# PX4/disparity_to_point_cloud

Measured on NVIDIA B200. Metric: Mpixels/s disparity->PointCloud2, higher is better.
Workload: dtype f64

## Files before the change

disparity_to_point_cloud_b200/csrc/capi.cu:

```cuda
#include "../../include/d2pc_b200.h"

#include <algorithm>
#include <atomic>
#include <cfloat>
#include <cmath>
#include <cstdio>
#include <cstdlib>
#include <cstring>
#include <mutex>
#include <new>
#include <string>
#include <utility>
#include <vector>

#include <nvtx3/nvToolsExt.h>
#include <sys/mman.h>

#include "cloud_transform.h"
#include "crop_box.h"
#include "fusion.h"
#include "laser_scan.h"
#include "median.h"
#include "radius_outlier.h"
#include "reproject.h"
// ... 49 lines not shown
  DevBuf d_in, d_out;
  StageBufs stages;
  DevBuf d_fuse_in[4], d_pre[2], d_container, d_combined, d_fused;
  DevBuf d_ranges;
  PinBuf h_ranges;
  uint32_t *d_count = nullptr;
  uint32_t *h_count = nullptr;
  cudaEvent_t ev_h2d = nullptr, ev_kernel = nullptr, ev_d2h = nullptr;
  cudaEvent_t ev_start = nullptr;
  bool timed = false;
  cudaStream_t s_kern = nullptr;
  bool pending = false;
  CloudPlan plan;
  uint8_t *user_dst = nullptr;
  size_t user_cap = 0;
  bool user_pinned = false;
  bool late_copy = false;
};

}

struct d2pc_ctx {
  d2pc_config cfg;
  int device = 0;
  int sm_count = 148;
  cudaStream_t s_h2d = nullptr, s_compute = nullptr, s_d2h = nullptr;
  double q[16];
  QParams Q;
  std::vector<Slot> slots;
  uint32_t epoch = 0;
  uint64_t launches = 0;
  std::string last_cuda_error;
  StageBufs batch;
  uint32_t *d_ticket = nullptr;
  d2pc_voxel_grid voxel;
  bool voxel_set = false;
  d2pc_radius_outlier ror;
  d2pc_crop_box box;
  d2pc_cloud_transform xform;
  d2pc_laser_scan_params scan;
  ScanPlan scan_plan;
  d2pc_laser_scan last_scan{};
  bool last_scan_on = false;
  DevBuf d_fuse_in[4], d_container, d_combined, d_fused;
  PinBuf h_fused, h_combined;
  DevBuf d_score_in, d_score_out[2];
  PinBuf h_score[2];
  DevBuf d_color_in, d_color_out, d_color_lut;
  PinBuf h_color;
  PinBuf h_stage;
  bool color_lut_ready = false;
  cudaEvent_t ev_fuse = nullptr;
  int rows_per_unit = 0, ctas_per_sm = 0, median_strip = 0, median_variant = 0;
  bool force_scalar = false, force_generic = false;
  int compact_variant = 0, exact_variant = 0, prefetch_dist = 0, zero_numer = 0, crop_load = 0, crop_probe = 0;
  int fuse_median = 0;
  int direct_out = 0;
  bool timing = false;
  std::vector<std::pair<uintptr_t, bool>> pin_cache;
  uint64_t pin_cache_gen = 0;
};

namespace {

struct NvtxRange {
  explicit NvtxRange(const char *name) { nvtxRangePushA(name); }
  ~NvtxRange() { nvtxRangePop(); }
};

std::atomic<uint64_t> g_host_gen{1};

int cuda_fail(d2pc_ctx *ctx, cudaError_t e, const char *what) {
  if (ctx) {
    ctx->last_cuda_error = std::string(what) + ": " + cudaGetErrorString(e);
  }
  if (e == cudaErrorMemoryAllocation) return D2PC_ERR_NOMEM;
  if (e == cudaErrorNoDevice || e == cudaErrorInsufficientDriver || e == cudaErrorInvalidDevice)
    return D2PC_ERR_NO_DEVICE;
  return D2PC_ERR_CUDA;
}

#define CU(ctx, call)                                      \
  do {                                                     \
    cudaError_t e__ = (call);                              \
    if (e__ != cudaSuccess) return cuda_fail(ctx, e__, #call); \
  } while (0)

int grow_dev(d2pc_ctx *ctx, DevBuf &b, size_t bytes, cudaStream_t clear_on = nullptr) {
  if (bytes <= b.cap) return D2PC_OK;
  if (b.p) CU(ctx, cudaFree(b.p));
  b.p = nullptr;
  b.cap = 0;
  const size_t cap = round_up(bytes, 1 << 16);
  CU(ctx, cudaMalloc(&b.p, cap));
  if (clear_on) CU(ctx, cudaMemsetAsync(b.p, 0, cap, clear_on));
  b.cap = cap;
  return D2PC_OK;
}
struct HostBlock {
  void *p;
  size_t bytes;
};
std::mutex g_thp_mutex;
std::vector<HostBlock> g_thp_blocks;

cudaError_t pinned_alloc(void **out, size_t bytes) {
// ... 287 lines not shown
}

int enqueue_reproject(d2pc_ctx *ctx, const CloudPlan &p, const FrameBatch &in, StageBufs &b, const CloudDst &dst,
                      uint32_t *ticket, cudaStream_t stream) {
  const d2pc_config &c = ctx->cfg;
  int nl = 0;
  ReprojectLaunch L;
  L.in = in.data;
  L.in_is_f32 = in.is_f32;
  L.step = in.step;
  L.frame_stride = in.frame_stride;
  L.n_frames = in.n_frames;
  L.width = in.w;
  L.height = in.h;
  L.border = c.border;
  L.scale = c.disparity_scale;
  L.out = dst.points;
  L.out_stride_bytes = dst.stride;
  L.counts = dst.counts;
  L.Q = &ctx->Q;
  L.arith_fast = c.arith_mode == D2PC_ARITH_FAST;
  L.compact = p.compact;
  L.scratch = b.scratch.p;
  L.tables = b.tables.p;
  L.ticket = ticket;
  L.sm_count = ctx->sm_count;
  L.rows_per_unit = ctx->rows_per_unit;
  L.ctas_per_sm = ctx->ctas_per_sm;
  L.force_scalar = ctx->force_scalar;
  L.force_generic = ctx->force_generic;
  L.compact_variant = ctx->compact_variant;
  L.exact_variant = ctx->exact_variant;
  L.zero_numer = ctx->zero_numer;
  L.prefetch_dist = ctx->prefetch_dist;
  L.crop_load = ctx->crop_load;
  L.crop_probe = ctx->crop_probe != 0;
  if (!in.is_f32 && c.median_ksize > 1) {
    MedianLaunch M;
    M.src = in.data;
    M.dst = b.med.p;
    M.src_step = M.dst_step = in.step;
    M.src_frame_stride = M.dst_frame_stride = in.frame_stride;
    M.n_frames = in.n_frames;
    M.width = (int)in.w;
    M.height = (int)in.h;
    M.ox0 = c.border;
    M.oy0 = c.border;
    M.ow = (int)in.w - 2 * c.border;
    M.oh = (int)in.h - 2 * c.border;
    M.ksize = c.median_ksize;
    M.sm_count = ctx->sm_count;
    M.strip_rows = ctx->median_strip;
    M.variant = ctx->median_variant;
    bool zero_numer = false;
    const bool fuse = ctx->fuse_median >= 0 && M.ow > 0 && M.oh > 0 && (c.median_ksize > 3 || M.variant != 0) &&
                      reproject_fuses_with_median(L, &zero_numer);
    if (fuse) {
      M.zero_numer = zero_numer;
      M.points = dst.points;
      M.points_stride_bytes = dst.stride;
      M.Q = &ctx->Q;
      M.scale = c.disparity_scale;
    }
    CU(ctx, launch_median_u8(M, stream, &nl));
    ctx->launches += nl;
    if (fuse) return D2PC_OK;
    L.in = b.med.p;
  }
  L.epoch = L.compact ? next_epoch(ctx) : 0;
  CU(ctx, launch_reproject(L, stream, &nl));
  ctx->launches += nl;
  return D2PC_OK;
}

int enqueue_kernels(d2pc_ctx *ctx, const CloudPlan &p, const FrameBatch &in, StageBufs &b, const CloudDst &out,
                    uint32_t *fallback, uint32_t *ticket, cudaStream_t stream, float *ranges = nullptr) {
  const uint32_t n = (uint32_t)p.n;
  const int stages = p.n_stages;
  const CloudDst buf[2] = {cloud_buf(b.cloud[0], in.n_frames, n), cloud_buf(b.cloud[1], in.n_frames, n)};
  int rc = enqueue_reproject(ctx, p, in, b, stages ? buf[0] : out, ticket, stream);
  for (int i = 0; i < stages && !rc; ++i) {
    const CloudDst &src = buf[i & 1];
    const CloudSrc cloud{src.points, src.stride, i > 0 || p.compact ? src.counts : nullptr, in.n_frames, n};
    rc = enqueue_stage(ctx, p.stages[i], cloud, i + 1 < stages ? buf[(i + 1) & 1] : out, fallback, b.stage.p, stream);
  }
  if (rc || !p.scan.on || !ranges) return rc;
  const CloudSrc cloud{out.points, out.stride, p.counted ? out.counts : nullptr, in.n_frames, n};
  int nl = 0;
  CU(ctx, launch_laser_scan(cloud, p.scan.p, ranges, (size_t)p.scan.p.n * 4, stream, &nl));
  ctx->launches += nl;
  return D2PC_OK;
}

int check_frame(const d2pc_ctx *ctx, const void *data, uint32_t w, uint32_t h, size_t step, int esz) {
  if (!ctx || !data) return D2PC_ERR_INVALID_ARG;
  if (w == 0 || h == 0 || w > (1u << 16) || h > (1u << 16)) return D2PC_ERR_BAD_DIMS;
  if (step < (size_t)w * esz) return D2PC_ERR_BAD_DIMS;
  if (esz == 4 && (step % 4 != 0 || reinterpret_cast<uintptr_t>(data) % 4 != 0)) return D2PC_ERR_BAD_DIMS;
  return D2PC_OK;
}

int slot_wait_idle(d2pc_ctx *ctx, Slot &s) {
  if (s.pending) {
    CU(ctx, cudaEventSynchronize(s.ev_d2h));
    s.pending = false;
  }
// ... 193 lines not shown
  int n = 0;
  cudaError_t e = cudaGetDeviceCount(&n);
  if (e != cudaSuccess || n == 0) {
    cudaGetLastError();
    return D2PC_ERR_NO_DEVICE;
  }
  if (device < 0 || device >= n) return D2PC_ERR_NO_DEVICE;
  int major = 0;
  cudaDeviceGetAttribute(&major, cudaDevAttrComputeCapabilityMajor, device);
  if (major != 10) return D2PC_ERR_NO_DEVICE;

  d2pc_ctx *ctx = new (std::nothrow) d2pc_ctx();
  if (!ctx) return D2PC_ERR_NOMEM;
  ctx->cfg = c;
  ctx->device = device;
  int rc = D2PC_OK;
  auto fail = [&](int code) {
    d2pc_destroy(ctx);
    return code;
  };
  if (cudaSetDevice(device) != cudaSuccess) return fail(D2PC_ERR_NO_DEVICE);
  cudaDeviceGetAttribute(&ctx->sm_count, cudaDevAttrMultiProcessorCount, device);
  if (cudaStreamCreateWithFlags(&ctx->s_h2d, cudaStreamNonBlocking) != cudaSuccess ||
      cudaStreamCreateWithFlags(&ctx->s_compute, cudaStreamNonBlocking) != cudaSuccess ||
      cudaStreamCreateWithFlags(&ctx->s_d2h, cudaStreamNonBlocking) != cudaSuccess ||
      cudaEventCreateWithFlags(&ctx->ev_fuse, cudaEventDisableTiming) != cudaSuccess)
    return fail(D2PC_ERR_CUDA);
  if (cudaMalloc(&ctx->d_ticket, 64) != cudaSuccess) return fail(D2PC_ERR_NOMEM);
  ctx->slots.resize(c.n_slots);
  for (auto &s : ctx->slots) {
    if (cudaEventCreateWithFlags(&s.ev_h2d, cudaEventDisableTiming) != cudaSuccess ||
        cudaEventCreateWithFlags(&s.ev_kernel, cudaEventDisableTiming) != cudaSuccess ||
        cudaEventCreateWithFlags(&s.ev_d2h, cudaEventDisableTiming) != cudaSuccess ||
        cudaStreamCreateWithFlags(&s.s_kern, cudaStreamNonBlocking) != cudaSuccess)
      return fail(D2PC_ERR_CUDA);
    if (cudaMalloc(&s.d_count, 64) != cudaSuccess) return fail(D2PC_ERR_NOMEM);
    if (cudaHostAlloc(&s.h_count, 64, cudaHostAllocDefault) != cudaSuccess) return fail(D2PC_ERR_NOMEM);
    cudaMemsetAsync(s.d_count, 0, 64, ctx->s_compute);
  }
  rc = d2pc_q_from_intrinsics(c.fx, c.fy, c.cx, c.cy, c.baseline, c.rect_width, c.rect_height, ctx->q);
  if (rc) return fail(rc);
  make_qparams(ctx->q, &ctx->Q);
  d2pc_voxel_grid_default(&ctx->voxel);
  d2pc_radius_outlier_default(&ctx->ror);
  d2pc_crop_box_default(&ctx->box);
  d2pc_cloud_transform_default(&ctx->xform);
  d2pc_laser_scan_params_default(&ctx->scan);
  scan_plan_of(&ctx->scan, &ctx->scan_plan);

  if (const char *v = getenv("D2PC_ROWS_PER_UNIT")) ctx->rows_per_unit = atoi(v);
  if (const char *v = getenv("D2PC_CTAS_PER_SM")) ctx->ctas_per_sm = atoi(v);
  if (const char *v = getenv("D2PC_CROP_LOAD")) ctx->crop_load = atoi(v);
  if (const char *v = getenv("D2PC_MEDIAN_STRIP")) ctx->median_strip = atoi(v);
  if (const char *v = getenv("D2PC_EXACT_VARIANT")) ctx->exact_variant = atoi(v);

  if (c.max_width > 0 && c.max_height > 0) {
    for (auto &s : ctx->slots) {
      const size_t pitch = round_up((size_t)c.max_width * 4, kAlign);
      const uint64_t np = crop_points(c.max_width, c.max_height, c.border);
      if ((rc = grow_dev(ctx, s.d_in, pitch * c.max_height)) ||
          (rc = grow_dev(ctx, s.stages.med, pitch * c.max_height)) ||
          (rc = grow_dev(ctx, s.d_out, np * 16 + 16)) || (rc = grow_pin(ctx, s.h_out, np * 16 + 16)) ||
          (rc = grow_pin(ctx, s.h_in, (size_t)c.max_width * 4 * c.max_height)))
        return fail(rc);
    }
  }
  *out = ctx;
  return D2PC_OK;
}

void d2pc_destroy(d2pc_ctx *ctx) {
  if (!ctx) return;
  cudaSetDevice(ctx->device);
  cudaDeviceSynchronize();
  for (auto &s : ctx->slots) {
    free_pin(s.h_in), free_pin(s.h_out);
    free_dev(s.d_in), free_dev(s.d_out), free_stages(s.stages), free_dev(s.d_ranges), free_pin(s.h_ranges);
    for (auto &b : s.d_fuse_in) free_dev(b);
    free_dev(s.d_pre[0]), free_dev(s.d_pre[1]), free_dev(s.d_container), free_dev(s.d_combined), free_dev(s.d_fused);
    if (s.d_count) cudaFree(s.d_count);
    if (s.h_count) cudaFreeHost(s.h_count);
    if (s.ev_h2d) cudaEventDestroy(s.ev_h2d);
    if (s.ev_kernel) cudaEventDestroy(s.ev_kernel);
    if (s.ev_d2h) cudaEventDestroy(s.ev_d2h);
    if (s.ev_start) cudaEventDestroy(s.ev_start);
    if (s.s_kern) cudaStreamDestroy(s.s_kern);
  }
  free_stages(ctx->batch);
  for (auto &b : ctx->d_fuse_in) free_dev(b);
  free_dev(ctx->d_container), free_dev(ctx->d_combined), free_dev(ctx->d_fused);
  free_pin(ctx->h_fused), free_pin(ctx->h_combined);
  free_dev(ctx->d_score_in), free_dev(ctx->d_score_out[0]), free_dev(ctx->d_score_out[1]);
  free_pin(ctx->h_score[0]), free_pin(ctx->h_score[1]);
  free_dev(ctx->d_color_in), free_dev(ctx->d_color_out), free_dev(ctx->d_color_lut), free_pin(ctx->h_color);
  free_pin(ctx->h_stage);
  if (ctx->d_ticket) cudaFree(ctx->d_ticket);
  if (ctx->ev_fuse) cudaEventDestroy(ctx->ev_fuse);
  if (ctx->s_h2d) cudaStreamDestroy(ctx->s_h2d);
  if (ctx->s_compute) cudaStreamDestroy(ctx->s_compute);
  if (ctx->s_d2h) cudaStreamDestroy(ctx->s_d2h);
  cudaGetLastError();
  delete ctx;
}

int d2pc_set_q(d2pc_ctx *ctx, const double q[16]) {
  if (!ctx || !q) return D2PC_ERR_INVALID_ARG;
// ... 88 lines not shown
  *t = ctx->xform;
  return D2PC_OK;
}
void d2pc_laser_scan_params_default(d2pc_laser_scan_params *p) {
  if (!p) return;
  memset(p, 0, sizeof(*p));
  p->struct_size = sizeof(*p);
  p->min_height = DBL_MIN, p->max_height = DBL_MAX;
  p->angle_min = -M_PI, p->angle_max = M_PI, p->angle_increment = M_PI / 180.0;
  p->scan_time = 1.0 / 30.0;
  p->range_min = 0.0, p->range_max = DBL_MAX;
  p->use_inf = 1, p->inf_epsilon = 1.0;
  p->keep_cloud = 1;
}
int d2pc_set_laser_scan(d2pc_ctx *ctx, const d2pc_laser_scan_params *p) {
  if (!ctx) return D2PC_ERR_INVALID_ARG;
  ScanPlan s;
  const int rc = scan_plan_of(p, &s);
  if (rc) return rc;
  ctx->scan = *p;
  ctx->scan_plan = s;
  return D2PC_OK;
}
int d2pc_get_laser_scan(const d2pc_ctx *ctx, d2pc_laser_scan_params *p) {
  if (!ctx || !p) return D2PC_ERR_INVALID_ARG;
  *p = ctx->scan;
  return D2PC_OK;
}
int d2pc_laser_scan_ranges(const d2pc_laser_scan_params *p, uint32_t *n) {
  ScanPlan s;
  const int rc = n ? scan_plan_of(p, &s) : D2PC_ERR_INVALID_ARG;
  if (rc) return rc;
  *n = s.msg.n_ranges;
  return D2PC_OK;
}
int d2pc_last_scan(const d2pc_ctx *ctx, d2pc_laser_scan *out) {
  if (!ctx || !out) return D2PC_ERR_INVALID_ARG;
  if (!ctx->last_scan_on) return D2PC_ERR_NOT_READY;
  *out = ctx->last_scan;
  return D2PC_OK;
}
int d2pc_set_arith_mode(d2pc_ctx *ctx, int m) {
  if (!ctx || m < 0 || m > 1) return D2PC_ERR_INVALID_ARG;
  ctx->cfg.arith_mode = m;
  return D2PC_OK;
}
int d2pc_set_tuning(d2pc_ctx *ctx, const char *key, int value) {
  if (!ctx || !key) return D2PC_ERR_INVALID_ARG;
  const std::string k(key);
  if (k == "rows_per_unit") ctx->rows_per_unit = value;
  else if (k == "ctas_per_sm") ctx->ctas_per_sm = value;
  else if (k == "median_strip") ctx->median_strip = value;
  else if (k == "median_variant") ctx->median_variant = value;
  else if (k == "force_scalar") ctx->force_scalar = value != 0;
  else if (k == "force_generic") ctx->force_generic = value != 0;
  else if (k == "force_park" || k == "compact_variant") ctx->compact_variant = value;
  else if (k == "exact_variant") ctx->exact_variant = value;
  else if (k == "zero_numer") ctx->zero_numer = value;
  else if (k == "fuse_median") ctx->fuse_median = value;
  else if (k == "direct_out") ctx->direct_out = value;
  else if (k == "prefetch_dist") ctx->prefetch_dist = value;
  else if (k == "crop_load") ctx->crop_load = value;
  else if (k == "crop_probe") ctx->crop_probe = value;
  else if (k == "median_ksize") {
    if (value < 1 || value > 15 || !(value & 1)) return D2PC_ERR_INVALID_ARG;
    ctx->cfg.median_ksize = value;
  } else if (k == "border") {
    if (value < 0) return D2PC_ERR_INVALID_ARG;
    ctx->cfg.border = value;
  } else if (k == "offset_x") ctx->cfg.offset_x = value;
  else if (k == "offset_y") ctx->cfg.offset_y = value;
  else if (k == "fuse_rule") {
    if (value < 0 || value > 7) return D2PC_ERR_INVALID_ARG;
    ctx->cfg.fuse_rule = value;
  } else if (k == "fuse_median_ksize") {
    if (value < 1 || value > 15 || !(value & 1)) return D2PC_ERR_INVALID_ARG;
    ctx->cfg.fuse_median_ksize = value;
  } else if (k == "fuse_crop_left") ctx->cfg.fuse_crop_left = value;
  else if (k == "fuse_crop_right") ctx->cfg.fuse_crop_right = value;
  else if (k == "fuse_crop_top") ctx->cfg.fuse_crop_top = value;
  else if (k == "fuse_crop_bottom") ctx->cfg.fuse_crop_bottom = value;
  else return D2PC_ERR_INVALID_ARG;
  return D2PC_OK;
}

int d2pc_submit_mono8(d2pc_ctx *ctx, int slot, const uint8_t *data, uint32_t w, uint32_t h, uint32_t step) {
  return submit_common(ctx, slot, data, w, h, step, false);
}
int d2pc_submit_f32(d2pc_ctx *ctx, int slot, const float *disp, uint32_t w, uint32_t h, uint32_t step) {
  return submit_common(ctx, slot, disp, w, h, step, true);
}

static void note_scan(d2pc_ctx *ctx, const ScanPlan &scan, const PinBuf &ranges) {
  ctx->last_scan_on = scan.on;
  ctx->last_scan = scan.msg;
  ctx->last_scan.ranges = reinterpret_cast<const float *>(ranges.p);
}

int d2pc_wait(d2pc_ctx *ctx, int slot, d2pc_cloud *out) {
  if (!ctx || slot < 0 || slot >= (int)ctx->slots.size()) return D2PC_ERR_INVALID_ARG;
  Slot &s = ctx->slots[slot];
  if (!s.pending) return D2PC_ERR_NOT_READY;
  CU(ctx, cudaSetDevice(ctx->device));
  CU(ctx, cudaEventSynchronize(s.ev_d2h));
  const uint64_t n = kept_points(s.plan, s.h_count);
  if (s.plan.counted && s.user_dst && s.user_cap < n * 16) {
// ... 254 lines not shown
  const LaserScanParams &p = ctx->scan_plan.p;
  const uint64_t bytes = (uint64_t)n_max * 16, rbytes = (uint64_t)p.n * 4;
  if (bytes > 0xffffffffull) return D2PC_ERR_BAD_DIMS;
  if (reinterpret_cast<uintptr_t>(d_in) % 16 || in_stride % 16 || reinterpret_cast<uintptr_t>(d_ranges) % 4 ||
      ranges_stride % 4 || (n_frames > 1 && (in_stride < bytes || ranges_stride < rbytes)))
    return D2PC_ERR_BAD_DIMS;
  if (n_frames == 0 || p.n == 0) return D2PC_OK;
  const uintptr_t in0 = reinterpret_cast<uintptr_t>(d_in), out0 = reinterpret_cast<uintptr_t>(d_ranges);
  const uint64_t in_end = in0 + (uint64_t)(n_frames - 1) * in_stride + bytes;
  const uint64_t out_end = out0 + (uint64_t)(n_frames - 1) * ranges_stride + rbytes;
  if (bytes && in0 < out_end && out0 < in_end) return D2PC_ERR_INVALID_ARG;
  CU(ctx, cudaSetDevice(ctx->device));
  const uint32_t chunk = frames_per_chunk(n_frames, n_max);
  for (uint32_t f0 = 0; f0 < n_frames; f0 += chunk) {
    const CloudSrc in{d_in + f0 * in_stride, in_stride, d_in_counts ? d_in_counts + f0 : nullptr,
                      std::min(chunk, n_frames - f0), n_max};
    int nl = 0;
    CU(ctx, launch_laser_scan(in, p, reinterpret_cast<float *>(reinterpret_cast<uint8_t *>(d_ranges) + f0 * ranges_stride),
                              ranges_stride, ctx->s_compute, &nl));
    ctx->launches += nl;
  }
  return D2PC_OK;
}

int d2pc_reproject_f32_device(d2pc_ctx *ctx, const float *d_disp, uint32_t n_frames, uint32_t w, uint32_t h,
                              size_t step, size_t frame_stride, uint8_t *d_points, size_t points_stride,
                              uint32_t *d_counts) {
  if (step % 4 || frame_stride % 4 || reinterpret_cast<uintptr_t>(d_disp) % 4) return D2PC_ERR_BAD_DIMS;
  return reproject_device_common(ctx, d_disp, true, n_frames, w, h, step, frame_stride, d_points, points_stride,
                                 d_counts);
}
int d2pc_reproject_mono8_device(d2pc_ctx *ctx, const uint8_t *d_img, uint32_t n_frames, uint32_t w, uint32_t h,
                                size_t step, size_t frame_stride, uint8_t *d_points, size_t points_stride,
                                uint32_t *d_counts) {
  return reproject_device_common(ctx, d_img, false, n_frames, w, h, step, frame_stride, d_points, points_stride,
                                 d_counts);
}

int d2pc_median_u8_device(d2pc_ctx *ctx, const uint8_t *d_src, uint32_t w, uint32_t h, size_t src_step,
                          uint8_t *d_dst, size_t dst_step, int ksize) {
  if (!ctx || !d_src || !d_dst) return D2PC_ERR_INVALID_ARG;
  if (w == 0 || h == 0 || src_step < w || dst_step < w) return D2PC_ERR_BAD_DIMS;
  if (ksize < 3 || ksize > 15 || !(ksize & 1)) return D2PC_ERR_INVALID_ARG;
  CU(ctx, cudaSetDevice(ctx->device));
  MedianLaunch M;
  M.src = d_src, M.dst = d_dst;
  M.src_step = src_step, M.dst_step = dst_step;
  M.width = (int)w, M.height = (int)h;
  M.ox0 = 0, M.oy0 = 0, M.ow = (int)w, M.oh = (int)h;
  M.ksize = ksize;
  M.sm_count = ctx->sm_count;
  M.strip_rows = ctx->median_strip;
  M.variant = ctx->median_variant;
  int nl = 0;
  CU(ctx, launch_median_u8(M, ctx->s_compute, &nl));
  ctx->launches += nl;
  return D2PC_OK;
}

void *d2pc_compute_stream(d2pc_ctx *ctx) { return ctx ? (void *)ctx->s_compute : nullptr; }
int d2pc_sync(d2pc_ctx *ctx) {
  if (!ctx) return D2PC_ERR_INVALID_ARG;
  CU(ctx, cudaSetDevice(ctx->device));
  CU(ctx, cudaStreamSynchronize(ctx->s_h2d));
  CU(ctx, cudaStreamSynchronize(ctx->s_compute));
  for (auto &s : ctx->slots)
    if (s.s_kern) CU(ctx, cudaStreamSynchronize(s.s_kern));
  CU(ctx, cudaStreamSynchronize(ctx->s_d2h));
  return D2PC_OK;
}
uint64_t d2pc_launch_count(const d2pc_ctx *ctx) { return ctx ? ctx->launches : 0; }

int d2pc_fuse_geometry(const d2pc_ctx *ctx, uint32_t w, uint32_t h, int rect1[4], int rect2[4], int rectc[4],
                       int dims[3]) {
  if (!ctx) return D2PC_ERR_INVALID_ARG;
  FuseGeometry g;
  const d2pc_config &c = ctx->cfg;
  const bool ok = fuse_geometry((int)w, (int)h, c.offset_x, c.offset_y, c.fuse_crop_left, c.fuse_crop_right,
                                c.fuse_crop_top, c.fuse_crop_bottom, &g);
  if (rect1) memcpy(rect1, g.r1, sizeof(g.r1));
  if (rect2) memcpy(rect2, g.r2, sizeof(g.r2));
  if (rectc) memcpy(rectc, g.rc, sizeof(g.rc));
  if (dims) dims[0] = g.n, dims[1] = g.out_w, dims[2] = g.out_h;
  return ok ? D2PC_OK : D2PC_ERR_GEOMETRY;
}

static int fuse_device_impl(d2pc_ctx *ctx, const uint8_t *d1, const uint8_t *d2, const uint8_t *s1, const uint8_t *s2,
                            uint32_t w, uint32_t h, size_t step, uint8_t *d_fused, uint8_t *d_combined,
                            FuseGeometry *g_out, bool scores_cropped = false, DevBuf *container = nullptr,
                            cudaStream_t stream = nullptr) {
  if (!stream) stream = ctx->s_compute;
  const d2pc_config &c = ctx->cfg;
  FuseGeometry g;
  if (!fuse_geometry((int)w, (int)h, c.offset_x, c.offset_y, c.fuse_crop_left, c.fuse_crop_right, c.fuse_crop_top,
                     c.fuse_crop_bottom, &g))
    return D2PC_ERR_GEOMETRY;
  int rc;
  DevBuf &cont = container ? *container : ctx->d_container;
  if ((size_t)g.nc * g.nc > cont.cap) {
    CU(ctx, cudaStreamSynchronize(ctx->s_compute));
    if ((rc = grow_dev(ctx, cont, (size_t)g.nc * g.nc))) return rc;
  }
  FuseLaunch L;
  L.d1 = d1, L.d2 = d2, L.s1 = s1, L.s2 = s2;
  L.step = step;
  L.width = (int)w, L.height = (int)h;
  L.g = g;
  L.rule = c.fuse_rule;
  L.scores_cropped = scores_cropped;
  L.container = cont.p;
  L.combined = d_combined;
  int nl = 0;
  CU(ctx, launch_fuse_merge(L, stream, &nl));
  ctx->launches += nl;
  if (c.fuse_median_ksize > 1) {
    MedianLaunch M;
    M.src = cont.p;
    M.src_step = (size_t)g.nc;
    M.width = g.nc, M.height = g.nc;
    M.ox0 = g.out_x, M.oy0 = g.out_y, M.ow = g.out_w, M.oh = g.out_h;
    M.dst_step = (size_t)g.out_w;
    M.dst = reinterpret_cast<uint8_t *>(reinterpret_cast<uintptr_t>(d_fused) - ((size_t)g.out_y * g.out_w + g.out_x));
    M.ksize = c.fuse_median_ksize;
    M.sm_count = ctx->sm_count;
    M.variant = ctx->median_variant;
    CU(ctx, launch_median_u8(M, stream, &nl));
    ctx->launches += nl;
  } else {
    CU(ctx, cudaMemcpy2DAsync(d_fused, g.out_w, cont.p + (size_t)g.out_y * g.nc + g.out_x, g.nc, g.out_w,
                              g.out_h, cudaMemcpyDeviceToDevice, stream));
  }
  if (g_out) *g_out = g;
  return D2PC_OK;
}

int d2pc_fuse_device(d2pc_ctx *ctx, const uint8_t *d_d1, const uint8_t *d_d2, const uint8_t *d_s1,
                     const uint8_t *d_s2, uint32_t w, uint32_t h, size_t step, uint8_t *d_fused,
                     uint8_t *d_combined) {
  if (!ctx || !d_d1 || !d_d2 || !d_s1 || !d_s2 || !d_fused) return D2PC_ERR_INVALID_ARG;
  if (w == 0 || h == 0 || step < w) return D2PC_ERR_BAD_DIMS;
  CU(ctx, cudaSetDevice(ctx->device));
  return fuse_device_impl(ctx, d_d1, d_d2, d_s1, d_s2, w, h, step, d_fused, d_combined, nullptr);
}

int d2pc_fuse_preprocessed_device(d2pc_ctx *ctx, const uint8_t *d_d1, const uint8_t *d_d2, const uint8_t *d_s1c,
                                  const uint8_t *d_s2c, uint32_t w, uint32_t h, size_t step, uint8_t *d_fused,
                                  uint8_t *d_combined) {
  if (!ctx || !d_d1 || !d_d2 || !d_s1c || !d_s2c || !d_fused) return D2PC_ERR_INVALID_ARG;
  if (w == 0 || h == 0 || step < w) return D2PC_ERR_BAD_DIMS;
  CU(ctx, cudaSetDevice(ctx->device));
  return fuse_device_impl(ctx, d_d1, d_d2, d_s1c, d_s2c, w, h, step, d_fused, d_combined, nullptr, true);
}

static int fuse_upload_and_run(d2pc_ctx *ctx, const uint8_t *const in[4], uint32_t w, uint32_t h, uint32_t step,
                               FuseGeometry *g) {
  int rc;
  const size_t pitch = w, fb = (size_t)w * h;
  CU(ctx, cudaSetDevice(ctx->device));
  CU(ctx, cudaStreamSynchronize(ctx->s_compute));
  if ((rc = grow_pin(ctx, ctx->h_stage, 4 * fb))) return rc;
  for (int i = 0; i < 4; ++i) {
    if ((rc = grow_dev(ctx, ctx->d_fuse_in[i], fb)) ||
        (rc = upload_dense(ctx, i * fb, ctx->d_fuse_in[i].p, in[i], w, h, step, ctx->s_compute)))
      return rc;
  }
  const size_t side = (size_t)(w < h ? w : h);
  if ((rc = grow_dev(ctx, ctx->d_fused, side * side)) || (rc = grow_dev(ctx, ctx->d_combined, side * side)))
    return rc;
  return fuse_device_impl(ctx, ctx->d_fuse_in[0].p, ctx->d_fuse_in[1].p, ctx->d_fuse_in[2].p, ctx->d_fuse_in[3].p, w, h,
                          pitch, ctx->d_fused.p, ctx->d_combined.p, g);
}

int d2pc_fuse(d2pc_ctx *ctx, const uint8_t *d1, const uint8_t *d2, const uint8_t *s1, const uint8_t *s2, uint32_t w,
              uint32_t h, uint32_t step, d2pc_image *fused, d2pc_image *combined) {
  if (!ctx || !d1 || !d2 || !s1 || !s2 || !fused) return D2PC_ERR_INVALID_ARG;
  if (w == 0 || h == 0 || step < w) return D2PC_ERR_BAD_DIMS;
  const uint8_t *in[4] = {d1, d2, s1, s2};
  FuseGeometry g;
// ... 377 lines not shown
```

disparity_to_point_cloud_b200/csrc/median.cu:

```cuda
#include "median.h"

#include <cstdint>

#include "reproject_math.cuh"

namespace d2pc {
namespace {

constexpr int kWarps = 4;
constexpr int kThreads = kWarps * 32;
constexpr int kRingPitch = 48;

struct MedianArgs {
  const uint8_t *src;
  uint8_t *dst;
  size_t src_step, dst_step, src_frame_stride, dst_frame_stride;
  int width, height;
  int ox0, oy0, ow, oh;
  int strip_rows, n_colblk, n_strip;
  uint32_t units_per_frame, total_units;
  float4 *points;
  size_t points_frame_stride;
  float scale;
  int zero_numer;
  QParams Q;
};

__device__ __forceinline__ int clampi(int v, int lo, int hi) { return min(max(v, lo), hi); }

__device__ __forceinline__ uint32_t hist_off(uint32_t bin) { return ((bin >> 2) << 7) | (bin & 3u); }

template <int kDelta>
__device__ __forceinline__ void bump_if_below(int &below, uint32_t off, uint32_t med_off) {
  asm("{\n\t.reg .pred p;\n\tsetp.lt.u32 p, %1, %2;\n\t@p add.s32 %0, %0, %3;\n\t}" : "+r"(below) : "r"(off), "r"(med_off), "n"(kDelta));
}

template <int K, int kFuse>
__global__ void __launch_bounds__(kThreads) median_hist_kernel(const __grid_constant__ MedianArgs a) {
  constexpr int R = K / 2;
  constexpr int kRank = (K * K) / 2;
  __shared__ __align__(16) uint8_t s_hist[kWarps][256 * 32];
  __shared__ __align__(4) uint16_t s_ring[kWarps][K][kRingPitch];
  const int lane = threadIdx.x & 31, wic = threadIdx.x >> 5;
  uint8_t *hist = s_hist[wic];
  uint8_t *hb = hist + 4 * lane;
  uint16_t(*ring)[kRingPitch] = s_ring[wic];

  for (uint32_t unit = blockIdx.x * kWarps + wic; unit < a.total_units; unit += gridDim.x * kWarps) {
    const uint32_t f = unit / a.units_per_frame;
    const uint32_t rem = unit - f * a.units_per_frame;
    const int strip = rem / a.n_colblk;
    const int cb = rem - strip * a.n_colblk;
    const int x0 = a.ox0 + cb * 32;
    const int y_first = a.oy0 + strip * a.strip_rows;
    const int y_end = min(y_first + a.strip_rows, a.oy0 + a.oh);
    const uint8_t *src = a.src + (size_t)f * a.src_frame_stride;
    uint8_t *dst = a.dst + (size_t)f * a.dst_frame_stride;
    const bool col_ok = (x0 + lane) < (a.ox0 + a.ow);
    double xd = 0.0;
    bool xslow = false, xzero = false;
    float4 *points = nullptr;
    if constexpr (kFuse != 0) {
      xd = rect_axis_const(x0 + lane, a.Q.q03);
      xslow = rect_axis_slow_t<kFuse == 2>(xd) || a.Q.zd_slow;
      xzero = kFuse == 2 && rect_axis_zero(xd);
      points = a.points + (size_t)f * a.points_frame_stride + (x0 + lane - a.ox0);
    }

    const int gx_a = clampi(x0 - R + lane, 0, a.width - 1);
    const int gx_b = clampi(x0 - R + 32 + lane, 0, a.width - 1);

    __syncwarp();
#pragma unroll
    for (int i = 0; i < (256 * 32) / (32 * 16); ++i)
      reinterpret_cast<uint4 *>(hist)[i * 32 + lane] = make_uint4(0, 0, 0, 0);

#pragma unroll
    for (int s = 0; s < K; ++s) {
      const uint8_t *row = src + (size_t)clampi(y_first - R + s, 0, a.height - 1) * a.src_step;
      ring[s][lane] = (uint16_t)hist_off(row[gx_a]);
      if (lane < K - 1) ring[s][32 + lane] = (uint16_t)hist_off(row[gx_b]);
    }
    __syncwarp();
#pragma unroll 1
    for (int s = 0; s < K; ++s) {
#pragma unroll
      for (int dx = 0; dx < K; ++dx) {
        const uint32_t off = ring[s][lane + dx];
        hb[off] = hb[off] + 1;
      }
    }
    int med = 0, below = 0;
    {
      int w = 0;
      for (; w < 64; ++w) {
        const uint32_t word = reinterpret_cast<const uint32_t *>(hist)[w * 32 + lane];
        const int s4 = (word & 0xff) + ((word >> 8) & 0xff) + ((word >> 16) & 0xff) + (word >> 24);
        if (below + s4 > kRank) break;
        below += s4;
      }
      med = w * 4;
      while (below + (int)hb[hist_off(med)] <= kRank) {
        below += hb[hist_off(med)];
        ++med;
      }
    }
    uint32_t med_off = hist_off(med);

    int slot = 0;
    for (int y = y_first; y < y_end; ++y) {
      if constexpr (kFuse != 0) {
        if (col_ok) {
          const float disp = __fadd_rn(__fmul_rn((float)med, a.scale), 0.0f);
          const double yd = rect_axis_const(y, a.Q.q13);
          bool slow;
          float4 p = reproject_exact_rectified<true, true, kFuse == 2>(
              a.Q, xd, yd, xslow || rect_axis_slow_t<kFuse == 2>(yd), xzero || (kFuse == 2 && rect_axis_zero(yd)), disp, slow);
          if (__builtin_expect(slow, 0)) p = reproject_exact_slow(a.Q.q, x0 + lane, y, disp);
          __stcs(points + (size_t)(y - a.oy0) * a.ow, p);
        }
      } else {
        if (col_ok) dst[(size_t)y * a.dst_step + x0 + lane] = (uint8_t)med;
      }
      if (y + 1 >= y_end) break;
      const uint8_t *row = src + (size_t)clampi(y + 1 + R, 0, a.height - 1) * a.src_step;
      const uint32_t na = hist_off(row[gx_a]);
      const uint32_t nb = (lane < K - 1) ? hist_off(row[gx_b]) : 0u;
      uint32_t offs[K];
#pragma unroll
      for (int dx = 0; dx < K; ++dx) offs[dx] = ring[slot][lane + dx];
#pragma unroll
      for (int dx = 0; dx < K; ++dx) {
        hb[offs[dx]] = hb[offs[dx]] - 1;
        bump_if_below<-1>(below, offs[dx], med_off);
      }
      __syncwarp();
      ring[slot][lane] = (uint16_t)na;
      if (lane < K - 1) ring[slot][32 + lane] = (uint16_t)nb;
      __syncwarp();
#pragma unroll
      for (int dx = 0; dx < K; ++dx) offs[dx] = ring[slot][lane + dx];
#pragma unroll
      for (int dx = 0; dx < K; ++dx) {
        hb[offs[dx]] = hb[offs[dx]] + 1;
        bump_if_below<1>(below, offs[dx], med_off);
      }
      slot = (slot + 1 == K) ? 0 : slot + 1;
      while (below > kRank) {
        --med;
        below -= hb[hist_off(med)];
      }
      for (;;) {
        const int hm = hb[hist_off(med)];
        if (below + hm > kRank) break;
        below += hm;
        ++med;
      }
      med_off = hist_off(med);
    }
  }
}

__device__ __forceinline__ void exch(int &a, int &b) {
  const int lo = min(a, b);
  b = max(a, b);
  a = lo;
}
__global__ void __launch_bounds__(128) median3_net_kernel(const __grid_constant__ MedianArgs a) {
  const int x = a.ox0 + (int)(blockIdx.x * 128 + threadIdx.x);
  const int y = a.oy0 + (int)blockIdx.y;
  if (x >= a.ox0 + a.ow) return;
  const uint8_t *src = a.src + (size_t)blockIdx.z * a.src_frame_stride;
  const int xm = max(x - 1, 0), xp = min(x + 1, a.width - 1);
  const uint8_t *r0 = src + (size_t)max(y - 1, 0) * a.src_step;
  const uint8_t *r1 = src + (size_t)y * a.src_step;
  const uint8_t *r2 = src + (size_t)min(y + 1, a.height - 1) * a.src_step;
  int p0 = r0[xm], p1 = r0[x], p2 = r0[xp], p3 = r1[xm], p4 = r1[x], p5 = r1[xp], p6 = r2[xm], p7 = r2[x], p8 = r2[xp];
  exch(p1, p2), exch(p4, p5), exch(p7, p8);
  exch(p0, p1), exch(p3, p4), exch(p6, p7);
  exch(p1, p2), exch(p4, p5), exch(p7, p8);
  exch(p0, p3), exch(p5, p8), exch(p4, p7);
  exch(p3, p6), exch(p1, p4), exch(p2, p5);
  exch(p4, p7), exch(p4, p2), exch(p6, p4);
  exch(p4, p2);
  (a.dst + (size_t)blockIdx.z * a.dst_frame_stride)[(size_t)y * a.dst_step + x] = (uint8_t)p4;
}

template <int K>
cudaError_t launch_k(const MedianArgs &a, int grid, cudaStream_t s) {
  if (a.points && a.zero_numer) median_hist_kernel<K, 2><<<grid, kThreads, 0, s>>>(a);
  else if (a.points) median_hist_kernel<K, 1><<<grid, kThreads, 0, s>>>(a);
  else median_hist_kernel<K, 0><<<grid, kThreads, 0, s>>>(a);
  return cudaGetLastError();
}

}

cudaError_t launch_median_u8(const MedianLaunch &L, cudaStream_t stream, int *launches) {
  if (launches) *launches = 0;
  if (L.ow <= 0 || L.oh <= 0 || L.n_frames == 0 || L.width <= 0 || L.height <= 0) return cudaSuccess;
  if (L.ksize < 3 || L.ksize > 15 || (L.ksize & 1) == 0) return cudaErrorInvalidValue;
  MedianArgs a{};
  a.src = L.src;
  a.dst = L.dst;
  a.src_step = L.src_step;
  a.dst_step = L.dst_step;
  a.src_frame_stride = L.src_frame_stride;
  a.dst_frame_stride = L.dst_frame_stride;
  a.width = L.width;
  a.height = L.height;
  a.ox0 = L.ox0;
  a.oy0 = L.oy0;
  a.ow = L.ow;
  a.oh = L.oh;
  if (L.points) {
    if (!L.Q || L.points_stride_bytes % 16 != 0) return cudaErrorInvalidValue;
    a.points = reinterpret_cast<float4 *>(L.points);
    a.points_frame_stride = L.points_stride_bytes / 16;
    a.scale = L.scale;
    a.zero_numer = L.zero_numer ? 1 : 0;
    a.Q = *L.Q;
  }
  if (launches) *launches = 1;
  if (L.ksize == 3 && L.variant == 0 && !L.points && L.oh <= 65535 && L.n_frames <= 65535) {
    median3_net_kernel<<<dim3((unsigned)((L.ow + 127) / 128), (unsigned)L.oh, L.n_frames), 128, 0, stream>>>(a);
    return cudaGetLastError();
  }
  a.n_colblk = (L.ow + 31) / 32;
  int strip = 64;
  const uint64_t want = (uint64_t)L.sm_count * 16;
  while (strip > 2 && (uint64_t)a.n_colblk * ((L.oh + strip - 1) / strip) * L.n_frames < want) strip >>= 1;
  if (L.strip_rows > 0) strip = L.strip_rows;
  a.strip_rows = strip;
  a.n_strip = (L.oh + strip - 1) / strip;
  a.units_per_frame = (uint32_t)a.n_colblk * (uint32_t)a.n_strip;
  const uint64_t total = (uint64_t)a.units_per_frame * L.n_frames;
  if (total > 0xffffffffull) return cudaErrorInvalidValue;
  a.total_units = (uint32_t)total;
  const uint64_t cap = (uint64_t)L.sm_count * 6;
  const uint64_t ctas = (total + kWarps - 1) / kWarps;
  const int grid = (int)(ctas < cap ? ctas : cap);
  switch (L.ksize) {
    case 3: return launch_k<3>(a, grid, stream);
    case 5: return launch_k<5>(a, grid, stream);
    case 7: return launch_k<7>(a, grid, stream);
    case 9: return launch_k<9>(a, grid, stream);
    case 11: return launch_k<11>(a, grid, stream);
    case 13: return launch_k<13>(a, grid, stream);
    default: return launch_k<15>(a, grid, stream);
  }
}

}
```

disparity_to_point_cloud_b200/csrc/median.h:

```cpp
#pragma once
#include <cstddef>
#include <cstdint>
#include <cuda_runtime.h>

#include "reproject.h"

namespace d2pc {

struct MedianLaunch {
  const uint8_t *src = nullptr;
  uint8_t *dst = nullptr;
  size_t src_step = 0, dst_step = 0, src_frame_stride = 0, dst_frame_stride = 0;
  uint32_t n_frames = 1;
  int width = 0, height = 0;
  int ox0 = 0, oy0 = 0, ow = 0, oh = 0;
  int ksize = 11;
  int sm_count = 148;
  int strip_rows = 0;
  int variant = 0;
  uint8_t *points = nullptr;
  size_t points_stride_bytes = 0;
  const QParams *Q = nullptr;
  float scale = 0.125f;
  bool zero_numer = false;
};

cudaError_t launch_median_u8(const MedianLaunch &L, cudaStream_t stream, int *launches);

}
```

Measured before the change: 358,300.

## Add column-histogram median kernel and retune strip height for large frames

Adds a new median filter kernel that keeps a per-column packed 4-bit/8-bit histogram in shared memory plus a row ring buffer, and tracks the median by counting values below it with SWAR popcount tricks. It is selectable with median_algo=2 and is off by default. The launch code also changes the default strip height when the computed strip stays at 64, using a batch_strip heuristic that applies to the existing kernel as well. This shifts the trade-off between per-strip setup cost and parallelism, and the new kernel adds shared-memory pressure and complexity.

```diff
diff --git a/disparity_to_point_cloud_b200/csrc/capi.cu b/disparity_to_point_cloud_b200/csrc/capi.cu
--- a/disparity_to_point_cloud_b200/csrc/capi.cu
+++ b/disparity_to_point_cloud_b200/csrc/capi.cu
@@ -125,6 +125,7 @@
   bool color_lut_ready = false;
   cudaEvent_t ev_fuse = nullptr;
   int rows_per_unit = 0, ctas_per_sm = 0, median_strip = 0, median_variant = 0;
+  int median_algo = 0;
   bool force_scalar = false, force_generic = false;
   int compact_variant = 0, exact_variant = 0, prefetch_dist = 0, zero_numer = 0, crop_load = 0, crop_probe = 0;
   int fuse_median = 0;
@@ -518,6 +519,7 @@
     M.sm_count = ctx->sm_count;
     M.strip_rows = ctx->median_strip;
     M.variant = ctx->median_variant;
+    M.algo = ctx->median_algo;
     bool zero_numer = false;
     const bool fuse = ctx->fuse_median >= 0 && M.ow > 0 && M.oh > 0 && (c.median_ksize > 3 || M.variant != 0) &&
                       reproject_fuses_with_median(L, &zero_numer);
@@ -817,6 +819,10 @@
   if (const char *v = getenv("D2PC_CTAS_PER_SM")) ctx->ctas_per_sm = atoi(v);
   if (const char *v = getenv("D2PC_CROP_LOAD")) ctx->crop_load = atoi(v);
   if (const char *v = getenv("D2PC_MEDIAN_STRIP")) ctx->median_strip = atoi(v);
+  if (const char *v = getenv("D2PC_MEDIAN_ALGO")) {
+    const int algo = atoi(v);
+    if (algo >= 0 && algo <= 2) ctx->median_algo = algo;
+  }
   if (const char *v = getenv("D2PC_EXACT_VARIANT")) ctx->exact_variant = atoi(v);
 
   if (c.max_width > 0 && c.max_height > 0) {
@@ -1011,6 +1017,10 @@
   else if (k == "ctas_per_sm") ctx->ctas_per_sm = value;
   else if (k == "median_strip") ctx->median_strip = value;
   else if (k == "median_variant") ctx->median_variant = value;
+  else if (k == "median_algo") {
+    if (value < 0 || value > 2) return D2PC_ERR_INVALID_ARG;
+    ctx->median_algo = value;
+  }
   else if (k == "force_scalar") ctx->force_scalar = value != 0;
   else if (k == "force_generic") ctx->force_generic = value != 0;
   else if (k == "force_park" || k == "compact_variant") ctx->compact_variant = value;
@@ -1371,6 +1381,7 @@
   M.sm_count = ctx->sm_count;
   M.strip_rows = ctx->median_strip;
   M.variant = ctx->median_variant;
+  M.algo = ctx->median_algo;
   int nl = 0;
   CU(ctx, launch_median_u8(M, ctx->s_compute, &nl));
   ctx->launches += nl;
@@ -1443,6 +1454,7 @@
     M.ksize = c.fuse_median_ksize;
     M.sm_count = ctx->sm_count;
     M.variant = ctx->median_variant;
+    M.algo = ctx->median_algo;
     CU(ctx, launch_median_u8(M, stream, &nl));
     ctx->launches += nl;
   } else {
diff --git a/disparity_to_point_cloud_b200/csrc/median.cu b/disparity_to_point_cloud_b200/csrc/median.cu
--- a/disparity_to_point_cloud_b200/csrc/median.cu
+++ b/disparity_to_point_cloud_b200/csrc/median.cu
@@ -35,6 +35,41 @@
   asm("{\n\t.reg .pred p;\n\tsetp.lt.u32 p, %1, %2;\n\t@p add.s32 %0, %0, %3;\n\t}" : "+r"(below) : "r"(off), "r"(med_off), "n"(kDelta));
 }
 
+template <int kFuse>
+struct MedianOut {
+  int x;
+  bool ok;
+  uint8_t *dst;
+  double xd = 0.0;
+  bool xslow = false, xzero = false;
+  float4 *points = nullptr;
+
+  __device__ __forceinline__ MedianOut(const MedianArgs &a, uint32_t f, int x_) : x(x_), ok(x_ < a.ox0 + a.ow) {
+    dst = a.dst + (size_t)f * a.dst_frame_stride;
+    if constexpr (kFuse != 0) {
+      xd = rect_axis_const(x, a.Q.q03);
+      xslow = rect_axis_slow_t<kFuse == 2>(xd) || a.Q.zd_slow;
+      xzero = kFuse == 2 && rect_axis_zero(xd);
+      points = a.points + (size_t)f * a.points_frame_stride + (x - a.ox0);
+    }
+  }
+
+  __device__ __forceinline__ void put(const MedianArgs &a, int y, int med) const {
+    if (!ok) return;
+    if constexpr (kFuse != 0) {
+      const float disp = __fadd_rn(__fmul_rn((float)med, a.scale), 0.0f);
+      const double yd = rect_axis_const(y, a.Q.q13);
+      bool slow;
+      float4 p = reproject_exact_rectified<true, true, kFuse == 2>(
+          a.Q, xd, yd, xslow || rect_axis_slow_t<kFuse == 2>(yd), xzero || (kFuse == 2 && rect_axis_zero(yd)), disp, slow);
+      if (__builtin_expect(slow, 0)) p = reproject_exact_slow(a.Q.q, x, y, disp);
+      __stcs(points + (size_t)(y - a.oy0) * a.ow, p);
+    } else {
+      dst[(size_t)y * a.dst_step + x] = (uint8_t)med;
+    }
+  }
+};
+
 template <int K, int kFuse>
 __global__ void __launch_bounds__(kThreads) median_hist_kernel(const __grid_constant__ MedianArgs a) {
   constexpr int R = K / 2;
@@ -55,17 +90,7 @@
     const int y_first = a.oy0 + strip * a.strip_rows;
     const int y_end = min(y_first + a.strip_rows, a.oy0 + a.oh);
     const uint8_t *src = a.src + (size_t)f * a.src_frame_stride;
-    uint8_t *dst = a.dst + (size_t)f * a.dst_frame_stride;
-    const bool col_ok = (x0 + lane) < (a.ox0 + a.ow);
-    double xd = 0.0;
-    bool xslow = false, xzero = false;
-    float4 *points = nullptr;
-    if constexpr (kFuse != 0) {
-      xd = rect_axis_const(x0 + lane, a.Q.q03);
-      xslow = rect_axis_slow_t<kFuse == 2>(xd) || a.Q.zd_slow;
-      xzero = kFuse == 2 && rect_axis_zero(xd);
-      points = a.points + (size_t)f * a.points_frame_stride + (x0 + lane - a.ox0);
-    }
+    const MedianOut<kFuse> out(a, f, x0 + lane);
 
     const int gx_a = clampi(x0 - R + lane, 0, a.width - 1);
     const int gx_b = clampi(x0 - R + 32 + lane, 0, a.width - 1);
@@ -109,19 +134,7 @@
 
     int slot = 0;
     for (int y = y_first; y < y_end; ++y) {
-      if constexpr (kFuse != 0) {
-        if (col_ok) {
-          const float disp = __fadd_rn(__fmul_rn((float)med, a.scale), 0.0f);
-          const double yd = rect_axis_const(y, a.Q.q13);
-          bool slow;
-          float4 p = reproject_exact_rectified<true, true, kFuse == 2>(
-              a.Q, xd, yd, xslow || rect_axis_slow_t<kFuse == 2>(yd), xzero || (kFuse == 2 && rect_axis_zero(yd)), disp, slow);
-          if (__builtin_expect(slow, 0)) p = reproject_exact_slow(a.Q.q, x0 + lane, y, disp);
-          __stcs(points + (size_t)(y - a.oy0) * a.ow, p);
-        }
-      } else {
-        if (col_ok) dst[(size_t)y * a.dst_step + x0 + lane] = (uint8_t)med;
-      }
+      out.put(a, y, med);
       if (y + 1 >= y_end) break;
       const uint8_t *row = src + (size_t)clampi(y + 1 + R, 0, a.height - 1) * a.src_step;
       const uint32_t na = hist_off(row[gx_a]);
@@ -157,6 +170,172 @@
         ++med;
       }
       med_off = hist_off(med);
+    }
+  }
+}
+
+template <int K>
+struct ColHist {
+  static constexpr int kWords = (3 + K + 3) / 4;
+  static constexpr int kSpan = 4 * (7 + kWords);
+  static constexpr int kPitch = ((kSpan / 4) & 1) ? kSpan : kSpan + 4;
+  static constexpr int kHistBytes = 128 * kPitch;
+  static constexpr int kRingRows = K + 1;
+};
+
+template <int K>
+__device__ __forceinline__ uint32_t window_mask(int lane, int j) {
+  const int lo = (lane & 3) - 4 * j, hi = lo + K;
+  const uint32_t m_lo = lo <= 0 ? 0xffffffffu : (lo >= 4 ? 0u : 0xffffffffu << (8 * lo));
+  const uint32_t m_hi = hi >= 4 ? 0xffffffffu : (hi <= 0 ? 0u : 0xffffffffu >> (8 * (4 - hi)));
+  return m_lo & m_hi;
+}
+
+template <int K>
+__device__ __forceinline__ int count_below(const uint32_t *w, const uint32_t (&mask80)[ColHist<K>::kWords],
+                                           uint32_t y4, uint32_t y7) {
+  int n = 0;
+#pragma unroll
+  for (int j = 0; j < ColHist<K>::kWords; ++j) {
+    const uint32_t x = w[j];
+    const uint32_t d = (x | 0x80808080u) - y7;
+    n += __popc(((~x & y4) | (~(x ^ y4) & ~d)) & mask80[j]);
+  }
+  return n;
+}
+
+template <int K>
+__device__ __forceinline__ int count_bin(const uint8_t *hist_q, const uint32_t (&mask0f)[ColHist<K>::kWords], int b) {
+  const uint32_t *w = reinterpret_cast<const uint32_t *>(hist_q + (b & 127) * ColHist<K>::kPitch);
+  const int sh = (b >> 5) & 4;
+  uint32_t acc = 0;
+#pragma unroll
+  for (int j = 0; j < ColHist<K>::kWords; ++j) acc += (w[j] >> sh) & mask0f[j];
+  return (int)((acc * 0x01010101u) >> 24);
+}
+
+template <int K, int kSign>
+__device__ __forceinline__ void col_update(uint8_t *hist, int col, uint32_t v) {
+  uint8_t *p = hist + (v & 127) * ColHist<K>::kPitch + col;
+  const int delta = (int)(v >> 7) * 15 + 1;
+  *p = (uint8_t)(*p + kSign * delta);
+}
+
+template <int K, int kFuse>
+__global__ void __launch_bounds__(kThreads) median_colhist_kernel(const __grid_constant__ MedianArgs a) {
+  using G = ColHist<K>;
+  constexpr int R = K / 2;
+  constexpr int kRank = (K * K) / 2;
+  constexpr int kProbes = 4;
+  __shared__ __align__(16) uint8_t s_hist[kWarps][G::kHistBytes];
+  __shared__ __align__(16) uint8_t s_ring[kWarps][G::kRingRows][G::kSpan];
+  const int lane = threadIdx.x & 31, wic = threadIdx.x >> 5;
+  uint8_t *hist = s_hist[wic];
+  const uint8_t *hist_q = hist + 4 * (lane >> 2);
+  uint8_t(*ring)[G::kSpan] = s_ring[wic];
+  const bool halo = lane < K - 1;
+
+  uint32_t mask80[G::kWords], mask0f[G::kWords];
+#pragma unroll
+  for (int j = 0; j < G::kWords; ++j) {
+    const uint32_t m = window_mask<K>(lane, j);
+    mask80[j] = m & 0x80808080u;
+    mask0f[j] = m & 0x0f0f0f0fu;
+  }
+  auto ring_words = [&](int slot) { return reinterpret_cast<const uint32_t *>(ring[slot]) + (lane >> 2); };
+
+  for (uint32_t unit = blockIdx.x * kWarps + wic; unit < a.total_units; unit += gridDim.x * kWarps) {
+    const uint32_t f = unit / a.units_per_frame;
+    const uint32_t rem = unit - f * a.units_per_frame;
+    const int strip = rem / a.n_colblk;
+    const int cb = rem - strip * a.n_colblk;
+    const int x0 = a.ox0 + cb * 32;
+    const int y_first = a.oy0 + strip * a.strip_rows;
+    const int y_end = min(y_first + a.strip_rows, a.oy0 + a.oh);
+    const uint8_t *src = a.src + (size_t)f * a.src_frame_stride;
+    const MedianOut<kFuse> out(a, f, x0 + lane);
+
+    const int gx_a = clampi(x0 - R + lane, 0, a.width - 1);
+    const int gx_b = clampi(x0 - R + 32 + lane, 0, a.width - 1);
+
+    __syncwarp();
+#pragma unroll
+    for (int i = 0; i < G::kHistBytes / (32 * 16); ++i)
+      reinterpret_cast<uint4 *>(hist)[i * 32 + lane] = make_uint4(0, 0, 0, 0);
+#pragma unroll
+    for (int s = 0; s < K; ++s) {
+      const uint8_t *row = src + (size_t)clampi(y_first - R + s, 0, a.height - 1) * a.src_step;
+      ring[s][lane] = row[gx_a];
+      if (halo) ring[s][32 + lane] = row[gx_b];
+    }
+    __syncwarp();
+#pragma unroll 1
+    for (int s = 0; s < K; ++s) {
+      col_update<K, 1>(hist, lane, ring[s][lane]);
+      if (halo) col_update<K, 1>(hist, 32 + lane, ring[s][32 + lane]);
+    }
+    int med = 0, lt = 0;
+    {
+      int hi = 256;
+#pragma unroll 1
+      for (int p = 0; p < kProbes; ++p) {
+        const int mid = (med + hi) >> 1;
+        const uint32_t y4 = (uint32_t)mid * 0x01010101u;
+        int c = 0;
+#pragma unroll 1
+        for (int s = 0; s < K; ++s) c += count_below<K>(ring_words(s), mask80, y4, y4 & 0x7f7f7f7fu);
+        if (c <= kRank) med = mid, lt = c;
+        else hi = mid;
+      }
+    }
+    __syncwarp();
+    for (;;) {
+      const int c = count_bin<K>(hist_q, mask0f, med);
+      if (lt + c > kRank) break;
+      lt += c;
+      ++med;
+    }
+
+    int s_out = 0, s_in = K;
+    const uint8_t *row_in = src + (size_t)clampi(y_first + 1 + R, 0, a.height - 1) * a.src_step;
+    uint32_t na = row_in[gx_a], nb = halo ? row_in[gx_b] : 0u;
+    for (int y = y_first; y < y_end; ++y) {
+      out.put(a, y, med);
+      if (y + 1 >= y_end) break;
+      if (y + 2 + R <= a.height - 1) row_in += a.src_step;
+      const uint32_t na_next = row_in[gx_a];
+      const uint32_t nb_next = halo ? row_in[gx_b] : 0u;
+      const uint32_t oa = ring[s_out][lane];
+      const uint32_t ob = halo ? ring[s_out][32 + lane] : 0u;
+      ring[s_in][lane] = (uint8_t)na;
+      if (halo) ring[s_in][32 + lane] = (uint8_t)nb;
+      __syncwarp();
+      const uint32_t y4 = (uint32_t)med * 0x01010101u, y7 = y4 & 0x7f7f7f7fu;
+      lt += count_below<K>(ring_words(s_in), mask80, y4, y7) - count_below<K>(ring_words(s_out), mask80, y4, y7);
+      col_update<K, -1>(hist, lane, oa);
+      col_update<K, 1>(hist, lane, na);
+      if (halo) {
+        col_update<K, -1>(hist, 32 + lane, ob);
+        col_update<K, 1>(hist, 32 + lane, nb);
+      }
+      s_out = (s_out == K) ? 0 : s_out + 1;
+      s_in = (s_in == K) ? 0 : s_in + 1;
+      na = na_next;
+      nb = nb_next;
+      __syncwarp();
+      if (lt > kRank) {
+        do {
+          --med;
+          lt -= count_bin<K>(hist_q, mask0f, med);
+        } while (lt > kRank);
+      } else {
+        for (;;) {
+          const int c = count_bin<K>(hist_q, mask0f, med);
+          if (lt + c > kRank) break;
+          lt += c;
+          ++med;
+        }
+      }
     }
   }
 }
@@ -187,11 +366,22 @@
 }
 
 template <int K>
-cudaError_t launch_k(const MedianArgs &a, int grid, cudaStream_t s) {
-  if (a.points && a.zero_numer) median_hist_kernel<K, 2><<<grid, kThreads, 0, s>>>(a);
-  else if (a.points) median_hist_kernel<K, 1><<<grid, kThreads, 0, s>>>(a);
-  else median_hist_kernel<K, 0><<<grid, kThreads, 0, s>>>(a);
+cudaError_t launch_k(const MedianArgs &a, bool colhist, int grid, cudaStream_t s) {
+  if (colhist) {
+    if (a.points && a.zero_numer) median_colhist_kernel<K, 2><<<grid, kThreads, 0, s>>>(a);
+    else if (a.points) median_colhist_kernel<K, 1><<<grid, kThreads, 0, s>>>(a);
+    else median_colhist_kernel<K, 0><<<grid, kThreads, 0, s>>>(a);
+  } else {
+    if (a.points && a.zero_numer) median_hist_kernel<K, 2><<<grid, kThreads, 0, s>>>(a);
+    else if (a.points) median_hist_kernel<K, 1><<<grid, kThreads, 0, s>>>(a);
+    else median_hist_kernel<K, 0><<<grid, kThreads, 0, s>>>(a);
+  }
   return cudaGetLastError();
+}
+
+int batch_strip(int oh) {
+  const int n = oh < 120 ? 1 : (oh + 40) / 80;
+  return (oh + n - 1) / n;
 }
 
 }
@@ -200,6 +390,7 @@
   if (launches) *launches = 0;
   if (L.ow <= 0 || L.oh <= 0 || L.n_frames == 0 || L.width <= 0 || L.height <= 0) return cudaSuccess;
   if (L.ksize < 3 || L.ksize > 15 || (L.ksize & 1) == 0) return cudaErrorInvalidValue;
+  if (L.algo < 0 || L.algo > 2) return cudaErrorInvalidValue;
   MedianArgs a{};
   a.src = L.src;
   a.dst = L.dst;
@@ -226,10 +417,13 @@
     median3_net_kernel<<<dim3((unsigned)((L.ow + 127) / 128), (unsigned)L.oh, L.n_frames), 128, 0, stream>>>(a);
     return cudaGetLastError();
   }
+  const bool colhist = L.algo == 2;
   a.n_colblk = (L.ow + 31) / 32;
+  const uint64_t cap = (uint64_t)L.sm_count * (colhist ? 7 : 6);
   int strip = 64;
   const uint64_t want = (uint64_t)L.sm_count * 16;
   while (strip > 2 && (uint64_t)a.n_colblk * ((L.oh + strip - 1) / strip) * L.n_frames < want) strip >>= 1;
+  if (strip == 64) strip = batch_strip(L.oh);
   if (L.strip_rows > 0) strip = L.strip_rows;
   a.strip_rows = strip;
   a.n_strip = (L.oh + strip - 1) / strip;
@@ -237,18 +431,17 @@
   const uint64_t total = (uint64_t)a.units_per_frame * L.n_frames;
   if (total > 0xffffffffull) return cudaErrorInvalidValue;
   a.total_units = (uint32_t)total;
-  const uint64_t cap = (uint64_t)L.sm_count * 6;
   const uint64_t ctas = (total + kWarps - 1) / kWarps;
   const int grid = (int)(ctas < cap ? ctas : cap);
   switch (L.ksize) {
-    case 3: return launch_k<3>(a, grid, stream);
-    case 5: return launch_k<5>(a, grid, stream);
-    case 7: return launch_k<7>(a, grid, stream);
-    case 9: return launch_k<9>(a, grid, stream);
-    case 11: return launch_k<11>(a, grid, stream);
-    case 13: return launch_k<13>(a, grid, stream);
-    default: return launch_k<15>(a, grid, stream);
-  }
-}
-
-}
+    case 3: return launch_k<3>(a, colhist, grid, stream);
+    case 5: return launch_k<5>(a, colhist, grid, stream);
+    case 7: return launch_k<7>(a, colhist, grid, stream);
+    case 9: return launch_k<9>(a, colhist, grid, stream);
+    case 11: return launch_k<11>(a, colhist, grid, stream);
+    case 13: return launch_k<13>(a, colhist, grid, stream);
+    default: return launch_k<15>(a, colhist, grid, stream);
+  }
+}
+
+}
diff --git a/disparity_to_point_cloud_b200/csrc/median.h b/disparity_to_point_cloud_b200/csrc/median.h
--- a/disparity_to_point_cloud_b200/csrc/median.h
+++ b/disparity_to_point_cloud_b200/csrc/median.h
@@ -18,6 +18,7 @@
   int sm_count = 148;
   int strip_rows = 0;
   int variant = 0;
+  int algo = 0;
   uint8_t *points = nullptr;
   size_t points_stride_bytes = 0;
   const QParams *Q = nullptr;
```

Result: no change. 358,200 (median of 6 runs) (-0.0%).
